# AmourWaltz/BayesLMs

Measured on AMD Instinct MI355X. Metric: train_tokens_per_sec, higher is better.
Workload: dtype f32

## Files before the change

### bayeslms_amd/csrc/blm_device.h

```cpp
#pragma once
#include <hip/hip_runtime.h>
#include <stdint.h>

#include "../../include/bayeslm.h"

#define BLM_WAVE 64

namespace blm {

struct u32x4 {
  uint32_t x, y, z, w;
};

__device__ __forceinline__ u32x4 philox4x32_10(uint32_t c0, uint32_t c1, uint32_t c2, uint32_t c3, uint32_t k0,
                                               uint32_t k1) {
  constexpr uint32_t M0 = 0xD2511F53u, M1 = 0xCD9E8D57u, W0 = 0x9E3779B9u, W1 = 0xBB67AE85u;
#pragma unroll
  for (int r = 0; r < 10; ++r) {
    const uint64_t p0 = (uint64_t)M0 * c0, p1 = (uint64_t)M1 * c2;
    const uint32_t hi0 = (uint32_t)(p0 >> 32), lo0 = (uint32_t)p0;
    const uint32_t hi1 = (uint32_t)(p1 >> 32), lo1 = (uint32_t)p1;
    const uint32_t n0 = hi1 ^ c1 ^ k0, n2 = hi0 ^ c3 ^ k1;
    c0 = n0; c1 = lo1; c2 = n2; c3 = lo0;
    k0 += W0; k1 += W1;
  }
  return {c0, c1, c2, c3};
}

__device__ __noinline__ u32x4 philox4x32_10_rolled(uint32_t c0, uint32_t c1, uint32_t c2, uint32_t c3, uint32_t k0,
                                                   uint32_t k1) {
  constexpr uint32_t M0 = 0xD2511F53u, M1 = 0xCD9E8D57u, W0 = 0x9E3779B9u, W1 = 0xBB67AE85u;
#pragma unroll 1
  for (int r = 0; r < 10; ++r) {
    const uint64_t p0 = (uint64_t)M0 * c0, p1 = (uint64_t)M1 * c2;
    const uint32_t hi0 = (uint32_t)(p0 >> 32), lo0 = (uint32_t)p0;
    const uint32_t hi1 = (uint32_t)(p1 >> 32), lo1 = (uint32_t)p1;
    const uint32_t n0 = hi1 ^ c1 ^ k0, n2 = hi0 ^ c3 ^ k1;
    c0 = n0; c1 = lo1; c2 = n2; c3 = lo0;
    k0 += W0; k1 += W1;
  }
  return {c0, c1, c2, c3};
}

__device__ __forceinline__ u32x4 philox_block(const blm_rng& r, uint64_t block) {
  return philox4x32_10((uint32_t)block, (uint32_t)(block >> 32), r.stream, r.step, (uint32_t)r.seed,
                       (uint32_t)(r.seed >> 32));
}

__device__ __forceinline__ void box_muller(uint32_t ra, uint32_t rb, float& z0, float& z1) {
  const float u1 = ((float)(ra >> 9) + 1.0f) * 1.1920928955078125e-07f;
  const float u2 = (float)(rb >> 8) * 5.9604644775390625e-08f;
  const float r = __builtin_sqrtf(-1.3862943611198906f * __builtin_amdgcn_logf(u1));
  z0 = r * __builtin_amdgcn_cosf(u2);
  z1 = r * __builtin_amdgcn_sinf(u2);
}

__device__ __forceinline__ float4 philox_normal4(const blm_rng& r, uint64_t block) {
  const u32x4 u = philox_block(r, block);
  float4 z;
  box_muller(u.x, u.y, z.x, z.y);
  box_muller(u.z, u.w, z.z, z.w);
  return z;
}

__device__ __forceinline__ float philox_normal1_rolled(const blm_rng& r, uint64_t idx) {
  const uint64_t block = idx >> 2;
  const u32x4 u = philox4x32_10_rolled((uint32_t)block, (uint32_t)(block >> 32), r.stream, r.step, (uint32_t)r.seed,
                                       (uint32_t)(r.seed >> 32));
  const bool hi = idx & 2;
  float z0, z1;
  box_muller(hi ? u.z : u.x, hi ? u.w : u.y, z0, z1);
  return (idx & 1) ? z1 : z0;
}
__device__ __forceinline__ uint32_t philox_bits1_rolled(const blm_rng& r, uint64_t idx) {
  const uint64_t block = idx >> 2;
  const u32x4 u = philox4x32_10_rolled((uint32_t)block, (uint32_t)(block >> 32), r.stream, r.step, (uint32_t)r.seed,
                                       (uint32_t)(r.seed >> 32));
  const int c = (int)(idx & 3);
  return c == 0 ? u.x : (c == 1 ? u.y : (c == 2 ? u.z : u.w));
}

__device__ __forceinline__ uint32_t dropout_threshold(float p) {
  const double t = (double)p * 4294967296.0;
  return t >= 4294967295.0 ? 0xFFFFFFFFu : (uint32_t)t;
}

__device__ __forceinline__ float wave_sum(float v) {
#pragma unroll
  for (int o = 32; o > 0; o >>= 1) v += __shfl_xor(v, o, 64);
  return v;
}
__device__ __forceinline__ float wave_max(float v) {
#pragma unroll
  for (int o = 32; o > 0; o >>= 1) v = fmaxf(v, __shfl_xor(v, o, 64));
  return v;
}

template <int NW>
__device__ __forceinline__ float block_sum(float v, float* red) {
  v = wave_sum(v);
  const int lane = threadIdx.x & 63, w = threadIdx.x >> 6;
  __syncthreads();
  if (lane == 0) red[w] = v;
  __syncthreads();
  float t = 0.f;
#pragma unroll
  for (int i = 0; i < NW; ++i) t += red[i];
  return t;
}
template <int NW>
__device__ __forceinline__ float block_max(float v, float* red) {
  v = wave_max(v);
  const int lane = threadIdx.x & 63, w = threadIdx.x >> 6;
  __syncthreads();
  if (lane == 0) red[w] = v;
  __syncthreads();
  float t = red[0];
#pragma unroll
  for (int i = 1; i < NW; ++i) t = fmaxf(t, red[i]);
  return t;
}

typedef float blm_f2 __attribute__((ext_vector_type(2)));
__device__ __forceinline__ void gelu_parts2(blm_f2 z, blm_f2& cdf, blm_f2& pdf_exp) {
  const blm_f2 x = __builtin_elementwise_abs(z) * 0.70710678118654752f;
  const blm_f2 den = __builtin_elementwise_fma(x, (blm_f2)(0.3275911f), (blm_f2)(1.0f));
  const blm_f2 t = {__builtin_amdgcn_rcpf(den.x), __builtin_amdgcn_rcpf(den.y)};
  const blm_f2 xx = -x * x;
  pdf_exp = (blm_f2){__expf(xx.x), __expf(xx.y)};
  blm_f2 poly = __builtin_elementwise_fma(t, (blm_f2)(1.061405429f), (blm_f2)(-1.453152027f));
  poly = __builtin_elementwise_fma(t, poly, (blm_f2)(1.421413741f));
  poly = __builtin_elementwise_fma(t, poly, (blm_f2)(-0.284496736f));
  poly = __builtin_elementwise_fma(t, poly, (blm_f2)(0.254829592f));
  const blm_f2 tail = (poly * t) * (0.5f * pdf_exp);
  cdf = (blm_f2){z.x >= 0.f ? 1.0f - tail.x : tail.x, z.y >= 0.f ? 1.0f - tail.y : tail.y};
}
__device__ __forceinline__ void gelu_parts(float z, float& cdf, float& pdf_exp) {
  const float x = fabsf(z) * 0.70710678118654752f;
  const float t = __builtin_amdgcn_rcpf(1.0f + 0.3275911f * x);
  pdf_exp = __expf(-x * x);
  const float poly = t * (0.254829592f + t * (-0.284496736f + t * (1.421413741f + t * (-1.453152027f + t * 1.061405429f))));
  const float tail = 0.5f * poly * pdf_exp;
  cdf = z >= 0.f ? 1.0f - tail : tail;
}
__device__ __forceinline__ float gelu_erf(float z) {
  float cdf, e;
  gelu_parts(z, cdf, e);
  return z * cdf;
}
__device__ __forceinline__ float dgelu_erf(float z) {
  float cdf, e;
  gelu_parts(z, cdf, e);
  return cdf + z * 0.3989422804014327f * e;
}

__device__ __forceinline__ float sigmoidf_(float x) { return 1.0f / (1.0f + __expf(-x)); }

__device__ __forceinline__ float gp_mix(float z, const float* coef, int N, int n) {
  return tanhf(z) * coef[n] + sigmoidf_(z) * coef[N + n] + fmaxf(z, 0.f) * coef[2 * N + n] +
         gelu_erf(z) * coef[3 * N + n];
}
__device__ __forceinline__ float dgp_mix(float z, const float* coef, int N, int n) {
  const float th = tanhf(z), sg = sigmoidf_(z);
  return (1.f - th * th) * coef[n] + sg * (1.f - sg) * coef[N + n] + (z > 0.f ? coef[2 * N + n] : 0.f) +
         dgelu_erf(z) * coef[3 * N + n];
}

}
```

### bayeslms_amd/csrc/gemm_f32_mfma.h

```cpp
#pragma once
#include <cstdlib>

#include "blm_device.h"
#include <type_traits>
#include "blm_host.h"

namespace blm {

using f32x16 = __attribute__((ext_vector_type(16))) float;

struct GemmP {
  int M, N, K;
  const float* A; long lda;
  const float* B; long ldb;
  float* C; long ldc;
  float alpha;
  unsigned flags;
  int epi;
  const float* bias;
  float* aux;
  const float* coef;
  blm_variational vb; int vb_cols;
  float* C2;
  const float* wg_mu;
// ... 183 lines not shown
  static constexpr int NREAD = ST64 ? 2 : 4;
  float v[4];
  f32x2 w[2];
  __device__ __forceinline__ void read(uint32_t base, int t) {
    if constexpr (ST64) {
#pragma unroll
      for (int h = 0; h < 2; ++h)
        asm volatile("ds_read2st64_b32 %0, %1 offset0:%2 offset1:%3" : "=v"(w[h]) : "v"(base), "n"((8 * t + 2 * h) * (S / 64)),
                     "n"((8 * t + 2 * h + 1) * (S / 64)));
    } else {
#pragma unroll
      for (int s = 0; s < 4; ++s) asm volatile("ds_read_b32 %0, %1 offset:%2" : "=v"(v[s]) : "v"(base), "n"((8 * t + s) * S * 4));
    }
  }
  __device__ __forceinline__ float get(int, int s) const {
    if constexpr (ST64) return (s & 1) ? w[s >> 1].y : w[s >> 1].x;
    else return v[s];
  }
  __device__ __forceinline__ void tie() {
    if constexpr (ST64) {
      asm volatile("" : "+v"(w[0]), "+v"(w[1]));
    } else {
#pragma unroll
      for (int s = 0; s < 4; ++s) asm volatile("" : "+v"(v[s]));
    }
  }
  __device__ __forceinline__ void add_k(f32x2 (&sum)[1]) {
    static_assert(ST64, "summed from the unpadded LDS-DMA images only");
    asm volatile("v_pk_add_f32 %0, %0, %1\n\tv_pk_add_f32 %0, %0, %2" : "+v"(sum[0]) : "v"(w[0]), "v"(w[1]));
  }
};
#ifndef BLM_GEMM_DMA
#define BLM_GEMM_DMA 1
#endif
template <int OP, int WTM, int WTN, bool SAMP, bool FAST>
constexpr bool use_dma() { return BLM_GEMM_DMA && !SAMP && FAST; }

template <int R>
__device__ __forceinline__ void r2s_kmaj_swz(float* tile, const float4 (&r)[R / 32]) {
  const int t = threadIdx.x, kq = t & 7, rr = t >> 3;
#pragma unroll
  for (int j = 0; j < R / 32; ++j) {
    const int row = rr + 32 * j;
    *reinterpret_cast<float4*>(tile + row * 32 + 4 * (kq ^ ((row >> 1) & 7))) = r[j];
  }
}

__device__ __forceinline__ void glds16(const float* gsrc, uint32_t lds_dst) {
  uint32_t keep;
  asm volatile("s_mov_b32 %0, m0\n\ts_mov_b32 m0, %2\n\ts_nop 0\n\tglobal_load_lds_dwordx4 %1, off\n\ts_mov_b32 m0, %0"
               : "=&s"(keep) : "v"(gsrc), "s"(lds_dst) : "memory");
}
__device__ __forceinline__ void glds16s(const float* sbase, uint32_t voff, uint32_t lds_dst) {
  uint32_t keep;
  asm volatile("s_mov_b32 %0, m0\n\ts_mov_b32 m0, %3\n\ts_nop 0\n\tglobal_load_lds_dwordx4 %1, %2\n\ts_mov_b32 m0, %0"
               : "=&s"(keep) : "v"(voff), "s"(sbase), "s"(lds_dst) : "memory");
}

template <int W> struct FragD {
  static constexpr int NREAD = W;
  f32x4 v[W];
  __device__ __forceinline__ void read(const uint32_t (&bt)[4], int t) {
#pragma unroll
    for (int i = 0; i < W; ++i) asm volatile("ds_read_b128 %0, %1 offset:%2" : "=v"(v[i]) : "v"(bt[t]), "n"(4096 * i));
  }
  __device__ __forceinline__ float get(int i, int s) const { return v[i][s]; }
  __device__ __forceinline__ void tie() {
#pragma unroll
    for (int i = 0; i < W; ++i) asm volatile("" : "+v"(v[i]));
  }
};

template <int N>
__device__ __forceinline__ void wait_lgkm() { asm volatile("s_waitcnt lgkmcnt(%0)" ::"n"(N > 15 ? 15 : N)); }

typedef __attribute__((ext_vector_type(2))) __bf16 bf16x2;
typedef __attribute__((ext_vector_type(8))) __bf16 bf16x8;
typedef __attribute__((ext_vector_type(4))) unsigned u32x4v;
__device__ __forceinline__ void split_bf16x8(const float (&x)[8], bf16x8& hi, bf16x8& lo) {
  u32x4v h, l;
#pragma unroll
  for (int q = 0; q < 4; ++q) {
    const f32x2 v = {x[2 * q], x[2 * q + 1]};
    const uint32_t hu = __builtin_bit_cast(uint32_t, __builtin_convertvector(v, bf16x2));
    const f32x2 r = {v.x - __uint_as_float(hu << 16), v.y - __uint_as_float(hu & 0xFFFF0000u)};
    h[q] = hu;
    l[q] = __builtin_bit_cast(uint32_t, __builtin_convertvector(r, bf16x2));
  }
  hi = __builtin_bit_cast(bf16x8, h);
  lo = __builtin_bit_cast(bf16x8, l);
}
__device__ __forceinline__ void split_bf16x8_3(const float (&x)[8], bf16x8& hi, bf16x8& mid, bf16x8& lo) {
  u32x4v h, m, l;
#pragma unroll
  for (int q = 0; q < 4; ++q) {
    const f32x2 v = {x[2 * q], x[2 * q + 1]};
    const bf16x2 hb = __builtin_convertvector(v, bf16x2);
    const f32x2 r = {v.x - (float)hb[0], v.y - (float)hb[1]};
    const bf16x2 mb = __builtin_convertvector(r, bf16x2);
    const f32x2 r2 = {r.x - (float)mb[0], r.y - (float)mb[1]};
    h[q] = __builtin_bit_cast(uint32_t, hb);
    m[q] = __builtin_bit_cast(uint32_t, mb);
    l[q] = __builtin_bit_cast(uint32_t, __builtin_convertvector(r2, bf16x2));
  }
  hi = __builtin_bit_cast(bf16x8, h);
  mid = __builtin_bit_cast(bf16x8, m);
  lo = __builtin_bit_cast(bf16x8, l);
}

__device__ __forceinline__ void gemm_keep_quad(const GemmP& p, int base_row, int row_stride, int col, float (&keep)[4]) {
  const int k = threadIdx.x & 3;
  const int m = base_row + k * row_stride;
  const int row = m / p.drop_B, b = m - row * p.drop_B;
  const uint64_t g = ((uint64_t)row * p.drop_global_cols + (uint64_t)(p.drop_col_offset + b)) * (uint64_t)p.N +
                     (uint64_t)(col & ~3);
  const u32x4 u = philox4x32_10_rolled((uint32_t)(g >> 2), (uint32_t)(g >> 34), p.drop_rng.stream, p.drop_rng.step,
                                       (uint32_t)p.drop_rng.seed, (uint32_t)(p.drop_rng.seed >> 32));
#define BLM_QUAD_BCAST(x, j) (uint32_t) __builtin_amdgcn_mov_dpp((int)(x), (j) * 0x55, 0xF, 0xF, true)
#define BLM_KEEP_FROM(j)                                                                                      \
  {                                                                                                           \
    const uint32_t w0 = BLM_QUAD_BCAST(u.x, j), w1 = BLM_QUAD_BCAST(u.y, j), w2 = BLM_QUAD_BCAST(u.z, j),     \
                   w3 = BLM_QUAD_BCAST(u.w, j);                                                               \
    const uint32_t w = k == 0 ? w0 : (k == 1 ? w1 : (k == 2 ? w2 : w3));                                      \
    keep[j] = w >= p.drop_thr ? p.drop_inv_keep : 0.f;                                                        \
  }
  BLM_KEEP_FROM(0) BLM_KEEP_FROM(1) BLM_KEEP_FROM(2) BLM_KEEP_FROM(3)
#undef BLM_KEEP_FROM
#undef BLM_QUAD_BCAST
}

__device__ __forceinline__ void gemm_keep_pair(const GemmP& p, int m, int c0, float& k0, float& k1) {
  const int row = m / p.drop_B, b = m - row * p.drop_B;
  const uint64_t g = ((uint64_t)row * p.drop_global_cols + (uint64_t)(p.drop_col_offset + b)) * (uint64_t)p.N + (uint64_t)c0;
  const u32x4 u = philox4x32_10_rolled((uint32_t)(g >> 2), (uint32_t)(g >> 34), p.drop_rng.stream, p.drop_rng.step,
                                       (uint32_t)p.drop_rng.seed, (uint32_t)(p.drop_rng.seed >> 32));
  const bool hi = g & 2;
  k0 = (hi ? u.z : u.x) >= p.drop_thr ? p.drop_inv_keep : 0.f;
  k1 = (hi ? u.w : u.y) >= p.drop_thr ? p.drop_inv_keep : 0.f;
}

__device__ __forceinline__ void gemm_eps_quad(const GemmP& p, int base_row, int row_stride, int col, float (&eps)[4]) {
  const int k = threadIdx.x & 3;
  const int rel = min(max(base_row + k * row_stride - p.vc.row_lo, 0), p.vc.srows - 1);
  const uint64_t si = (uint64_t)rel * (uint64_t)p.N + (uint64_t)(min(col, p.N - 1) & ~3);
  const u32x4 u = philox4x32_10_rolled((uint32_t)(si >> 2), (uint32_t)(si >> 34), p.vc.rng.stream, p.vc.rng.step,
                                       (uint32_t)p.vc.rng.seed, (uint32_t)(p.vc.rng.seed >> 32));
  float z0, z1, z2, z3;
  box_muller(u.x, u.y, z0, z1);
  box_muller(u.z, u.w, z2, z3);
#define BLM_QUAD_BCASTF(x, j) __int_as_float(__builtin_amdgcn_mov_dpp(__float_as_int(x), (j) * 0x55, 0xF, 0xF, true))
#define BLM_EPS_FROM(j)                                                                                   \
  {                                                                                                       \
    const float w0 = BLM_QUAD_BCASTF(z0, j), w1 = BLM_QUAD_BCASTF(z1, j), w2 = BLM_QUAD_BCASTF(z2, j),     \
                w3 = BLM_QUAD_BCASTF(z3, j);                                                              \
    eps[j] = k == 0 ? w0 : (k == 1 ? w1 : (k == 2 ? w2 : w3));                                            \
  }
  BLM_EPS_FROM(0) BLM_EPS_FROM(1) BLM_EPS_FROM(2) BLM_EPS_FROM(3)
#undef BLM_EPS_FROM
#undef BLM_QUAD_BCASTF
}

template <int EPI>
__device__ __forceinline__ void epi_elem(const GemmP& p, bool accum, int row, int col, float acc, float bias, float keep, bool kl_on = true, bool atomic = false) {
  const long o = (long)row * p.ldc + col;
  float v = p.alpha * acc;
  if constexpr (EPI == BLM_EPI_BIAS) {
    if (kl_on) v += bias;
  } else if constexpr (EPI == BLM_EPI_BIAS_GELU) {
    v += bias;
    float cdf, e;
    gelu_parts(v, cdf, e);
    if (p.aux) p.aux[o] = (cdf + v * 0.3989422804014327f * e) * keep;
    v = v * cdf * keep;
  } else if constexpr (EPI == BLM_EPI_MUL_DGELU) {
    v *= p.aux[o];
  } else if constexpr (EPI == BLM_EPI_GP_MIX) {
    v += bias;
    if (p.aux) p.aux[o] = v;
    v = gp_mix(v, p.coef, p.N, col) * keep;
  } else if constexpr (EPI == BLM_EPI_MUL_DGP_MIX) {
    v *= keep;
    if (p.C2) p.C2[o] = v;
    v *= dgp_mix(p.aux[o], p.coef, p.N, col);
  } else if constexpr (EPI == BLM_EPI_BAYES_WGRAD) {
    const float dW = v;
    const int rel = row - p.vc.row_lo;
    if ((unsigned)rel < (unsigned)p.vc.srows) {
      const long si = (long)rel * p.N + col;
      const float sig = __expf(p.vc.lgstd[si]);
      float e;
      if (p.vc.eps) e = p.vc.eps[si];
      else if (p.eps_quad) e = keep;
      else e = philox_normal1_rolled(p.vc.rng, (uint64_t)si);
      const float klw = kl_on ? p.kl_lambda * p.kl_inv_n : 0.f;
      const float g2 = dW * e * sig + klw * (sig * sig - 1.0f);
      if (atomic) atomicAdd(p.C2 + si, g2);
      else p.C2[si] = accum ? p.C2[si] + g2 : g2;
      v = dW + klw * p.wg_mu[o];
    }
  }
  if constexpr (EPI == BLM_EPI_NONE || EPI == BLM_EPI_BIAS || EPI == BLM_EPI_BAYES_WGRAD) {
    if (atomic) { atomicAdd(p.C + o, v); return; }
  }
  p.C[o] = accum ? p.C[o] + v : v;
}

template <int EPI, int WTM, int WTN>
__device__ __forceinline__ void epilogue(const GemmP& p, f32x16 (&acc)[WTM][WTN], int m0, int n0, int wm, int wn,
                                         int li, int lh, bool kl_on = true, bool atomic = false) {
  constexpr bool DROP = (EPI == BLM_EPI_BIAS_GELU || EPI == BLM_EPI_GP_MIX || EPI == BLM_EPI_MUL_DGP_MIX);
  constexpr bool BIAS = (EPI == BLM_EPI_BIAS || EPI == BLM_EPI_BIAS_GELU || EPI == BLM_EPI_GP_MIX);
  const bool accum = p.flags & BLM_GEMM_ACCUMULATE;
  int col[WTN];
  float bias[WTN];
#pragma unroll
  for (int j = 0; j < WTN; ++j) {
    col[j] = n0 + wn * (32 * WTN) + ((INTERLEAVE && WTN == 2) ? 2 * li + j : 32 * j + li);
    bias[j] = 0.f;
    if constexpr (BIAS) bias[j] = col[j] < p.N ? p.bias[col[j]] : 0.f;
  }
  const bool pair_store = INTERLEAVE && WTN == 2 && (EPI == BLM_EPI_NONE || EPI == BLM_EPI_BIAS) && !atomic && (p.ldc % 2 == 0) &&
                          ((reinterpret_cast<uintptr_t>(p.C) & 7) == 0);
#pragma unroll
  for (int i = 0; i < WTM; ++i) {
#pragma unroll
    for (int rq = 0; rq < 4; ++rq) {
      const int mrow0 = 8 * rq + 4 * lh;
      const int row0 = m0 + wm * (32 * WTM) + ((INTERLEAVE && WTM == 2) ? 2 * mrow0 + i : 32 * i + mrow0);
      constexpr int RS = (INTERLEAVE && WTM == 2) ? 2 : 1;
      float keep[4][WTN];
#pragma unroll
      for (int rr = 0; rr < 4; ++rr)
#pragma unroll
        for (int j = 0; j < WTN; ++j) keep[rr][j] = 1.f;
      if constexpr (EPI == BLM_EPI_BAYES_WGRAD) {
        if (p.eps_quad) {
#pragma unroll
          for (int j = 0; j < WTN; ++j) {
            float e4[4];
            gemm_eps_quad(p, row0, RS, col[j], e4);
#pragma unroll
            for (int rr = 0; rr < 4; ++rr) keep[rr][j] = e4[rr];
          }
        }
      }
      if constexpr (DROP) {
        if (p.drop_on) {
          if (INTERLEAVE && WTN == 2 && p.drop_quad) {
#pragma unroll
            for (int rr = 0; rr < 4; ++rr) gemm_keep_pair(p, row0 + rr * RS, min(col[0], p.N - 2), keep[rr][0], keep[rr][WTN - 1]);
          } else if (!(INTERLEAVE && WTN == 2) && p.drop_quad) {
#pragma unroll
            for (int j = 0; j < WTN; ++j) {
              float k4[4];
              gemm_keep_quad(p, row0, RS, col[j], k4);
#pragma unroll
              for (int rr = 0; rr < 4; ++rr) keep[rr][j] = k4[rr];
            }
          } else {
#pragma unroll
            for (int rr = 0; rr < 4; ++rr)
#pragma unroll
              for (int j = 0; j < WTN; ++j) keep[rr][j] = gemm_keep(p, row0 + rr * RS, min(col[j], p.N - 1));
          }
        }
      }
#pragma unroll
      for (int rr = 0; rr < 4; ++rr) {
        const int row = row0 + rr * RS;
        const int r = 4 * rq + rr;
        if (row >= p.M) continue;
        if constexpr (WTN == 2) {
          if (pair_store && col[1] < p.N) {
            float2* dst = reinterpret_cast<float2*>(p.C + (long)row * p.ldc + col[0]);
            float2 v = make_float2(p.alpha * acc[i][0][r] + bias[0], p.alpha * acc[i][1][r] + bias[1]);
            if (accum) { const float2 old = *dst; v.x += old.x; v.y += old.y; }
            *dst = v;
            continue;
          }
        }
#pragma unroll
        for (int j = 0; j < WTN; ++j)
          if (col[j] < p.N) epi_elem<EPI>(p, accum, row, col[j], acc[i][j][r], bias[j], keep[rr][j], kl_on, atomic);
      }
    }
  }
  BLM_PROF_WG_END();
}

__device__ __forceinline__ void store4(float* dst, const float4& v) { *reinterpret_cast<float4*>(dst) = v; }

template <int EPI, int WTM, int WTN, int WGN = 2>
__device__ __forceinline__ void epilogue_rows(const GemmP& p, f32x16 (&acc)[WTM][WTN], float* stage, int m0, int n0,
                                              int wm, int wn, int li, int lh) {
  constexpr int BN = 32 * WTN * WGN, SS = BN + 4;
  constexpr int NP = WTM == 2 ? 2 : 1;
  constexpr int TPRW = BN / 4, RPS = (128 * WGN) / TPRW;
  const int t = threadIdx.x, c4 = 4 * (t % TPRW);
  const int col = n0 + c4;
  const bool accum = p.flags & BLM_GEMM_ACCUMULATE;
  float4 bias = make_float4(0.f, 0.f, 0.f, 0.f);
  if constexpr (EPI == BLM_EPI_BIAS || EPI == BLM_EPI_BIAS_GELU || EPI == BLM_EPI_GP_MIX || EPI == BLM_EPI_CE_PART || EPI == BLM_EPI_MC_PART)
    if (col < p.N && p.bias) bias = *reinterpret_cast<const float4*>(p.bias + col);
#pragma unroll
  for (int pass = 0; pass < NP; ++pass) {
    __syncthreads();
    if (WTM == 1 || wm == pass) {
#pragma unroll
      for (int i = 0; i < WTM; ++i)
#pragma unroll
        for (int j = 0; j < WTN; ++j)
#pragma unroll
          for (int r = 0; r < 16; ++r) {
            const int lrow = (WTM == 2 ? 32 * i : 32 * wm) + (r & 3) + 8 * (r >> 2) + 4 * lh;
            stage[lrow * SS + wn * (32 * WTN) + 32 * j + li] = p.alpha * acc[i][j][r];
          }
    }
    __syncthreads();
    if constexpr (EPI == BLM_EPI_CE_PART) {
      const bool valid = col < p.ce_nv;
      const bool part = valid && col + 4 > p.ce_nv;
      for (int lr = t / TPRW; lr < 64; lr += RPS) {
        const int row = m0 + 64 * pass + lr;
        if (row >= p.M) break;
        float4 v = *reinterpret_cast<const float4*>(stage + lr * SS + c4);
        v.x += bias.x; v.y += bias.y; v.z += bias.z; v.w += bias.w;
        if (part) {
          if (col + 1 >= p.ce_nv) v.y = -INFINITY;
          if (col + 2 >= p.ce_nv) v.z = -INFINITY;
          v.w = -INFINITY;
        }
        float m = valid ? fmaxf(fmaxf(v.x, v.y), fmaxf(v.z, v.w)) : -INFINITY;
#pragma unroll
        for (int o = TPRW / 2; o > 0; o >>= 1) m = fmaxf(m, __shfl_xor(m, o, 64));
        float sum = valid ? (__expf(v.x - m) + __expf(v.y - m)) + (__expf(v.z - m) + __expf(v.w - m)) : 0.f;
#pragma unroll
        for (int o = TPRW / 2; o > 0; o >>= 1) sum += __shfl_xor(sum, o, 64);
        if (t % TPRW == 0) {
          float* d = p.aux + ((long)row * p.gn + n0 / BN) * 2;
          d[0] = m;
          d[1] = sum;
        }
        const long long tg = p.ce_tgt[row >> p.ce_row_shift];
        if (valid && tg >= col && tg < col + 4 && tg < p.ce_nv) p.ce_tlogit[row] = tg == col ? v.x : (tg == col + 1 ? v.y : (tg == col + 2 ? v.z : v.w));
      }
    } else if constexpr (EPI == BLM_EPI_MC_PART) {
      const int sh = p.ce_row_shift, S = p.mc_s;
      const bool keep = p.epi == BLM_EPI_MC_LOGP;
      const float logS = __logf((float)S);
      const bool valid = col < p.ce_nv;
      const bool in1 = col + 1 < p.ce_nv, in2 = col + 2 < p.ce_nv, in3 = col + 3 < p.ce_nv;
      for (int g = t / TPRW; g < (64 >> sh); g += RPS) {
        const int row0 = m0 + 64 * pass + (g << sh);
        if (row0 >= p.M) break;
        float hs = 0.f, ms = 0.f;
        if (valid) {
          const float* z = stage + (g << sh) * SS + c4;
          const float* lse = p.mc_lse + row0;
          float4 r = make_float4(-INFINITY, -INFINITY, -INFINITY, -INFINITY);
          for (int s = 0; s < S; ++s) {
            const float4 v = *reinterpret_cast<const float4*>(z + s * SS);
            const float l = lse[s];
            r.x = fmaxf(r.x, v.x + bias.x - l); r.y = fmaxf(r.y, v.y + bias.y - l);
            r.z = fmaxf(r.z, v.z + bias.z - l); r.w = fmaxf(r.w, v.w + bias.w - l);
          }
          float4 sw = make_float4(0.f, 0.f, 0.f, 0.f), su = sw;
          for (int s = 0; s < S; ++s) {
            const float4 v = *reinterpret_cast<const float4*>(z + s * SS);
            const float l = lse[s];
            const float ux = v.x + bias.x - l - r.x, uy = v.y + bias.y - l - r.y, uz = v.z + bias.z - l - r.z, uw = v.w + bias.w - l - r.w;
            const float wx = __expf(ux), wy = __expf(uy), wz = __expf(uz), ww = __expf(uw);
            sw.x += wx; sw.y += wy; sw.z += wz; sw.w += ww;
            su.x = fmaf(wx, ux, su.x); su.y = fmaf(wy, uy, su.y); su.z = fmaf(wz, uz, su.z); su.w = fmaf(ww, uw, su.w);
          }
          const float invS = 1.f / S;
          auto col_terms = [&](float rr, float W, float U, bool in) {
            const float L = __logf(W) - logS, er = __expf(rr);
            if (in) {
              hs = fmaf(er * W * invS, rr + L, hs);
              ms = fmaf(er, fmaf(-L, W, U), ms);
            }
            return rr + L;
          };
          float4 lp;
          lp.x = col_terms(r.x, sw.x, su.x, true);
          lp.y = col_terms(r.y, sw.y, su.y, in1);
          lp.z = col_terms(r.z, sw.z, su.z, in2);
          lp.w = col_terms(r.w, sw.w, su.w, in3);
          if (keep) {
            float* d = p.C + (long)(row0 >> sh) * p.ldc + col;
            if (in3) {
              store4(d, lp);
            } else {
              d[0] = lp.x;
              if (in1) d[1] = lp.y;
              if (in2) d[2] = lp.z;
            }
          }
        }
#pragma unroll
        for (int o = TPRW / 2; o > 0; o >>= 1) {
          hs += __shfl_xor(hs, o, 64);
          ms += __shfl_xor(ms, o, 64);
        }
        if (t % TPRW == 0) {
          float* d = p.aux + ((long)(row0 >> sh) * p.gn + n0 / BN) * 2;
          d[0] = hs;
          d[1] = ms;
        }
      }
    } else if (col < p.N) {
      auto keep4 = [&](int row) {
        float4 kp = make_float4(1.f, 1.f, 1.f, 1.f);
        if (p.drop_on) {
          const int rr = row / p.drop_B, b = row - rr * p.drop_B;
          const uint64_t g = ((uint64_t)rr * p.drop_global_cols + (uint64_t)(p.drop_col_offset + b)) * (uint64_t)p.N + (uint64_t)col;
          const u32x4 u = philox4x32_10((uint32_t)(g >> 2), (uint32_t)(g >> 34), p.drop_rng.stream, p.drop_rng.step,
                                        (uint32_t)p.drop_rng.seed, (uint32_t)(p.drop_rng.seed >> 32));
          kp = make_float4(u.x >= p.drop_thr ? p.drop_inv_keep : 0.f, u.y >= p.drop_thr ? p.drop_inv_keep : 0.f,
                           u.z >= p.drop_thr ? p.drop_inv_keep : 0.f, u.w >= p.drop_thr ? p.drop_inv_keep : 0.f);
        }
        return kp;
      };
      auto row_body = [&](int lr, const float4& a) {
        const int row = m0 + 64 * pass + lr;
        float4 v = *reinterpret_cast<const float4*>(stage + lr * SS + c4);
        const long o = (long)row * p.ldc + col;
        if constexpr (EPI == BLM_EPI_BIAS) {
          v.x += bias.x; v.y += bias.y; v.z += bias.z; v.w += bias.w;
        } else if constexpr (EPI == BLM_EPI_GP_MIX) {
          const float4 kp = keep4(row);
          v.x += bias.x; v.y += bias.y; v.z += bias.z; v.w += bias.w;
          if (p.aux) store4(p.aux + o, v);
          v.x = gp_mix(v.x, p.coef, p.N, col) * kp.x;
          v.y = gp_mix(v.y, p.coef, p.N, col + 1) * kp.y;
          v.z = gp_mix(v.z, p.coef, p.N, col + 2) * kp.z;
          v.w = gp_mix(v.w, p.coef, p.N, col + 3) * kp.w;
        } else if constexpr (EPI == BLM_EPI_MUL_DGP_MIX) {
          const float4 kp = keep4(row);
          v.x *= kp.x; v.y *= kp.y; v.z *= kp.z; v.w *= kp.w;
          if (p.C2) store4(p.C2 + o, v);
          v.x *= dgp_mix(a.x, p.coef, p.N, col);
          v.y *= dgp_mix(a.y, p.coef, p.N, col + 1);
          v.z *= dgp_mix(a.z, p.coef, p.N, col + 2);
          v.w *= dgp_mix(a.w, p.coef, p.N, col + 3);
        } else if constexpr (EPI == BLM_EPI_BIAS_GELU) {
          const float4 kp = keep4(row);
          float4 d;
          {
            const blm_f2 z0 = (blm_f2){v.x, v.y} + (blm_f2){bias.x, bias.y}, z1 = (blm_f2){v.z, v.w} + (blm_f2){bias.z, bias.w};
            const blm_f2 k0 = {kp.x, kp.y}, k1 = {kp.z, kp.w};
            blm_f2 c0, e0, c1, e1;
            gelu_parts2(z0, c0, e0);
            gelu_parts2(z1, c1, e1);
            const blm_f2 d0 = __builtin_elementwise_fma(z0 * 0.3989422804014327f, e0, c0) * k0, y0 = (z0 * c0) * k0;
            const blm_f2 d1 = __builtin_elementwise_fma(z1 * 0.3989422804014327f, e1, c1) * k1, y1 = (z1 * c1) * k1;
            d = make_float4(d0.x, d0.y, d1.x, d1.y);
            v = make_float4(y0.x, y0.y, y1.x, y1.y);
          }
          if (p.aux) store4(p.aux + o, d);
        } else if constexpr (EPI == BLM_EPI_MUL_DGELU) {
          v.x *= a.x; v.y *= a.y; v.z *= a.z; v.w *= a.w;
        }
        float4* dst = reinterpret_cast<float4*>(p.C + o);
        if (accum) { const float4 old = *dst; v.x += old.x; v.y += old.y; v.z += old.z; v.w += old.w; }
#ifdef BLM_GEMM_LIFE
        if (blm_dbg_store == 1) { if (v.x == 1.2345e-30f) store4(p.C + o, v); return; }
        if (blm_dbg_store == 2) { store4(p.C + (long)(lr + 64 * pass) * p.ldc + c4, v); return; }
#endif
        store4(p.C + o, v);
      };
      if constexpr (EPI == BLM_EPI_MUL_DGELU || EPI == BLM_EPI_MUL_DGP_MIX) {
        constexpr int NIT = 64 / RPS;
        float4 ax[NIT];
#pragma unroll
        for (int i = 0; i < NIT; ++i) {
          const int row = m0 + 64 * pass + t / TPRW + RPS * i;
          ax[i] = row < p.M ? *reinterpret_cast<const float4*>(p.aux + (long)row * p.ldc + col) : make_float4(0.f, 0.f, 0.f, 0.f);
        }
#pragma unroll
        for (int i = 0; i < NIT; ++i) {
          const int lr = t / TPRW + RPS * i;
          if (m0 + 64 * pass + lr < p.M) row_body(lr, ax[i]);
        }
      } else {
        const float4 none = make_float4(0.f, 0.f, 0.f, 0.f);
        for (int lr = t / TPRW; lr < 64; lr += RPS) {
          if (m0 + 64 * pass + lr >= p.M) break;
          row_body(lr, none);
        }
      }
    }
  }
  BLM_PROF_WG_END();
}

template <int OP, int WTM, int WTN, bool SAMP, bool FAST, int SPLIT = 0, int WGN = 2>
__global__ __launch_bounds__(128 * WGN, WGN == 2 ? 2 : 1) void gemm_f32_kernel(const GemmP p) {
  constexpr int BM = 64 * WTM, BN = 32 * WTN * WGN, NT = 128 * WGN;
  constexpr bool A_KMAJ = (OP != BLM_GEMM_TN), B_KMAJ = (OP == BLM_GEMM_NT);
  constexpr bool DMA = use_dma<OP, WTM, WTN, SAMP, FAST>();
  constexpr int SA = BM + (DMA ? 0 : 4), SB = BN + (DMA ? 0 : 4);
  constexpr int KSX = DMA ? 32 : KS;
  constexpr int TA = A_KMAJ ? BM * KSX : BK * SA, TB = B_KMAJ ? BN * KSX : BK * SB;
  constexpr int NA = BM / 32, NB = BN / 32;
  extern __shared__ __attribute__((aligned(16))) float smem[];
  float* const As = smem;
  float* const Bs = smem + 2 * TA;

  const int nb = p.gm * p.gn;
  const bool whole = (int)blockIdx.x < p.tail_from;
  const int ntail = nb - p.tail_from, rtail = (int)blockIdx.x - p.tail_from;
  const int bid = whole ? (int)blockIdx.x : p.tail_from + rtail % ntail, ks = whole ? 0 : rtail / ntail;
  const bool atomic = p.atomic && !whole;
  const int q = nb >> 3, rem = nb & 7, xcd = bid & 7;
  const int id = (xcd < rem ? xcd * (q + 1) : rem * (q + 1) + (xcd - rem) * q) + (bid >> 3);
  constexpr int GROUP = 8;
  int mt, nt;
  if (p.gn <= GROUP) {
    mt = id / p.gn;
    nt = id - mt * p.gn;
  } else {
    const int per = GROUP * p.gn, grp = id / per, first = grp * GROUP, gsz = min(p.gm - first, GROUP), in = id - grp * per;
    mt = first + in % gsz;
    nt = in / gsz;
  }
  const int m0 = mt * BM, n0 = nt * BN;

  const int t = threadIdx.x, lane = t & 63, wave = t >> 6;
  const int wm = wave / WGN, wn = wave % WGN, li = lane & 31, lh = lane >> 5;
#ifdef BLM_GEMM_LIFE
  if (t == 0 && blockIdx.x < 8192) {
    blm_wg_life[4 * blockIdx.x] = wall_clock64();
    blm_wg_life[4 * blockIdx.x + 2] = (long long)__builtin_amdgcn_s_getreg((31 << 11) | 4) |
                                      ((long long)__builtin_amdgcn_s_getreg((31 << 11) | 20) << 32);
  }
#endif

  float4 ra[NA], rb[NB], rl[SAMP ? NB : 1];
  const float* pa[FAST ? NA : 1];
  const float* pb[FAST ? NB : 1];
  const float* pl[(FAST && SAMP) ? NB : 1];
  bool in_slice[(FAST && SAMP) ? NB : 1];
  long stepA = 0, stepB = 0, stepL = 0;

  if constexpr (FAST) {
    if constexpr (A_KMAJ) {
#pragma unroll
      for (int j = 0; j < NA; ++j) pa[j] = p.A + (long)min(m0 + (t >> 3) + 32 * j, p.M - 1) * p.lda + 4 * (t & 7);
      stepA = BK;
    } else {
      constexpr int TPR = BM / 4, RPP = 256 / TPR;
#pragma unroll
      for (int j = 0; j < NA; ++j) pa[j] = p.A + (long)(t / TPR + RPP * j) * p.lda + min(m0 + 4 * (t % TPR), p.M - 4);
      stepA = (long)BK * p.lda;
    }
    if constexpr (B_KMAJ) {
#pragma unroll
      for (int j = 0; j < NB; ++j) {
        const int n = min(n0 + (t >> 3) + 32 * j, p.N - 1);
        pb[j] = p.B + (long)n * p.ldb + 4 * (t & 7);
        if constexpr (SAMP) {
          const int rel = n - p.vb.row_lo;
          in_slice[j] = (unsigned)rel < (unsigned)p.vb.srows;
          pl[j] = p.vb.lgstd + (long)min(max(rel, 0), p.vb.srows - 1) * p.vb_cols + 4 * (t & 7);
        }
      }
      stepB = BK;
      stepL = BK;
    } else {
      constexpr int TPR = BN / 4, RPP = 256 / TPR;
#pragma unroll
      for (int j = 0; j < NB; ++j) {
        const int c = min(n0 + 4 * (t % TPR), p.N - 4);
        pb[j] = p.B + (long)(t / TPR + RPP * j) * p.ldb + c;
        if constexpr (SAMP) pl[j] = p.vb.lgstd + c;
      }
      stepB = (long)BK * p.ldb;
    }
  }

  float4 cs = make_float4(0.f, 0.f, 0.f, 0.f);
  const bool do_cs = !A_KMAJ && p.colsum_a != nullptr && n0 == 0;

  auto fetch_fast = [&](int kt) {
    if constexpr (FAST) {
#pragma unroll
      for (int j = 0; j < NA; ++j) ra[j] = *reinterpret_cast<const float4*>(pa[j] + kt * stepA);
#pragma unroll
      for (int j = 0; j < NB; ++j) rb[j] = *reinterpret_cast<const float4*>(pb[j] + kt * stepB);
      if constexpr (SAMP) {
        if constexpr (B_KMAJ) {
#pragma unroll
          for (int j = 0; j < NB; ++j) rl[j] = *reinterpret_cast<const float4*>(pl[j] + kt * stepL);
        } else {
          constexpr int TPR = BN / 4, RPP = 256 / TPR;
#pragma unroll
          for (int j = 0; j < NB; ++j) {
            const int rel = kt * BK + t / TPR + RPP * j - p.vb.row_lo;
            in_slice[j] = (unsigned)rel < (unsigned)p.vb.srows;
            rl[j] = *reinterpret_cast<const float4*>(pl[j] + (long)min(max(rel, 0), p.vb.srows - 1) * p.vb_cols);
          }
        }
      }
    }
  };
  auto fetch_slow = [&](int k0) {
    const bool av = p.a_vec, bv = p.b_vec;
    if constexpr (A_KMAJ) g2r_kmaj<BM>(p.A, p.lda, m0, p.M, k0, p.K, av, ra);
    else g2r_nmaj<BM>(p.A, p.lda, k0, p.K, m0, p.M, av, ra);
    if constexpr (B_KMAJ) g2r_kmaj<BN>(p.B, p.ldb, n0, p.N, k0, p.K, bv, rb);
    else g2r_nmaj<BN>(p.B, p.ldb, k0, p.K, n0, p.N, bv, rb);
    if constexpr (SAMP) {
      if constexpr (B_KMAJ) g2r_kmaj<BN>(p.vb.lgstd, p.vb_cols, n0 - p.vb.row_lo, p.vb.srows, k0, p.K, true, rl);
      else g2r_nmaj<BN>(p.vb.lgstd, p.vb_cols, k0 - p.vb.row_lo, p.vb.srows, n0, p.N, true, rl);
    }
  };
  auto stash = [&](int buf, int k0, bool fast) {
    float* At = As + buf * TA;
    float* Bt = Bs + buf * TB;
    if constexpr (SAMP) {
#pragma unroll
      for (int j = 0; j < NB; ++j) {
        int srow, scol;
        if constexpr (B_KMAJ) { srow = n0 + (t >> 3) + 32 * j; scol = k0 + 4 * (t & 7); }
        else { constexpr int TPR = BN / 4, RPP = 256 / TPR; srow = k0 + t / TPR + RPP * j; scol = n0 + 4 * (t % TPR); }
        if constexpr (FAST) {
          if (fast) {
            if constexpr (B_KMAJ) srow = min(srow, p.N - 1); else scol = min(scol, p.N - 4);
            if (in_slice[j]) rb[j] = sample4(rb[j], rl[j], p.vb, p.vb_cols, srow, scol);
            continue;
          }
        }
        rb[j] = sample4(rb[j], rl[j], p.vb, p.vb_cols, srow, scol);
      }
    }
    if constexpr (!A_KMAJ && !DMA) {
      if (do_cs) {
#pragma unroll
        for (int j = 0; j < NA; ++j) { cs.x += ra[j].x; cs.y += ra[j].y; cs.z += ra[j].z; cs.w += ra[j].w; }
      }
    }
    if constexpr (DMA) {
      if constexpr (A_KMAJ) r2s_kmaj_swz<BM>(At, ra); else r2s_nmaj<BM, SA>(At, ra);
      if constexpr (B_KMAJ) r2s_kmaj_swz<BN>(Bt, rb); else r2s_nmaj<BN, SB>(Bt, rb);
    } else {
      if constexpr (A_KMAJ) r2s_kmaj<BM>(At, ra); else r2s_nmaj<BM, SA>(At, ra);
      if constexpr (B_KMAJ) r2s_kmaj<BN>(Bt, rb); else r2s_nmaj<BN, SB>(Bt, rb);
    }
  };

  f32x16 acc[WTM][WTN];
#pragma unroll
  for (int i = 0; i < WTM; ++i)
#pragma unroll
    for (int j = 0; j < WTN; ++j) acc[i][j] = (f32x16)(0.f);

  auto compute = [&](int cur, auto&& mid) {
    using FA = FragG<A_KMAJ, WTM, SA>;
    using FB = FragG<B_KMAJ, WTN, SB>;
    const uint32_t a_base = A_KMAJ ? lds_u32(As + cur * TA + (wm * (32 * WTM) + li) * KS + 4 * lh)
                                   : lds_u32(As + cur * TA + (4 * lh) * SA + wm * (32 * WTM) + li);
    const uint32_t b_base = B_KMAJ ? lds_u32(Bs + cur * TB + (wn * (32 * WTN) + li) * KS + 4 * lh)
                                   : lds_u32(Bs + cur * TB + (4 * lh) * SB + wn * (32 * WTN) + li);
    FA a[2];
    FB b[2];
    a[0].read(a_base, 0);
    b[0].read(b_base, 0);
#pragma unroll
    for (int t4 = 0; t4 < 4; ++t4) {
      if (t4 + 1 < 4) {
        a[(t4 + 1) & 1].read(a_base, t4 + 1);
        b[(t4 + 1) & 1].read(b_base, t4 + 1);
        wait_lgkm<FA::NREAD + FB::NREAD>();
      } else {
        wait_lgkm<0>();
      }
      a[t4 & 1].tie();
      b[t4 & 1].tie();
      if (t4 == 2) mid();
      __builtin_amdgcn_sched_barrier(0);
#pragma unroll
      for (int s4 = 0; s4 < 4; ++s4)
#pragma unroll
        for (int i = 0; i < WTM; ++i)
#pragma unroll
          for (int j = 0; j < WTN; ++j)
            acc[i][j] = __builtin_amdgcn_mfma_f32_32x32x2f32(a[t4 & 1].get(i, s4), b[t4 & 1].get(j, s4), acc[i][j], 0, 0, 0);
    }
  };

  const int swz = (li >> 1) & 7;
  constexpr bool CS_FRAG = DMA && !A_KMAJ && SPLIT == 0, CS_WALK = DMA && !A_KMAJ && SPLIT != 0;
  struct CsOff {};
  struct CsPartials { f32x2 p[WTM]; int wn; };
  typename std::conditional<CS_FRAG, CsPartials, CsOff>::type csf;
  if constexpr (CS_FRAG) {
#pragma unroll
    for (int i = 0; i < WTM; ++i) csf.p[i] = (f32x2)(0.f);
    csf.wn = do_cs ? __builtin_amdgcn_readfirstlane(wn) : -1;
  }
  typename std::conditional<CS_WALK, float, CsOff>::type cs1{};
  auto compute_dma = [&](int cur) {
    if constexpr (DMA) {
      if constexpr (CS_WALK) {
        if (do_cs && t < BM) {
          const float* col = As + cur * TA + t;
#pragma unroll 8
          for (int k = 0; k < BK; ++k) cs1 += col[k * SA];
        }
      }
      using FA = typename std::conditional<A_KMAJ, FragD<WTM>, FragG<false, WTM, SA>>::type;
      using FB = typename std::conditional<B_KMAJ, FragD<WTN>, FragG<false, WTN, SB>>::type;
      uint32_t abt[4], bbt[4];
      const uint32_t a0 = A_KMAJ ? lds_u32(As + cur * TA + (wm * (32 * WTM) + li) * 32) : lds_u32(As + cur * TA + (4 * lh) * SA + wm * (32 * WTM) + li);
      const uint32_t b0 = B_KMAJ ? lds_u32(Bs + cur * TB + (wn * (32 * WTN) + li) * 32) : lds_u32(Bs + cur * TB + (4 * lh) * SB + wn * (32 * WTN) + li);
#pragma unroll
      for (int t4 = 0; t4 < 4; ++t4) {
        const uint32_t ch = (uint32_t)(((2 * t4 + lh) ^ swz) * 16);
        abt[t4] = a0 + ch;
        bbt[t4] = b0 + ch;
      }
      auto rd_a = [&](FA& f, int t4) { if constexpr (A_KMAJ) f.read(abt, t4); else f.read(a0, t4); };
      auto rd_b = [&](FB& f, int t4) { if constexpr (B_KMAJ) f.read(bbt, t4); else f.read(b0, t4); };
      if constexpr (SPLIT != 0) {
        FA a[4];
        FB b[4];
        rd_a(a[0], 0); rd_b(b[0], 0); rd_a(a[1], 1); rd_b(b[1], 1);
        rd_a(a[2], 2); rd_b(b[2], 2); rd_a(a[3], 3); rd_b(b[3], 3);
#pragma unroll
        for (int g = 0; g < 2; ++g) {
          constexpr int PEND = 2 * (FA::NREAD + FB::NREAD);
          if (g == 0) wait_lgkm<(PEND > 15 ? 15 : PEND)>(); else wait_lgkm<0>();
          a[2 * g].tie(); a[2 * g + 1].tie(); b[2 * g].tie(); b[2 * g + 1].tie();
          float xa[WTM][8], xb[WTN][8];
#pragma unroll
          for (int i = 0; i < WTM; ++i)
#pragma unroll
            for (int s4 = 0; s4 < 4; ++s4) { xa[i][s4] = a[2 * g].get(i, s4); xa[i][4 + s4] = a[2 * g + 1].get(i, s4); }
#pragma unroll
          for (int j = 0; j < WTN; ++j)
#pragma unroll
            for (int s4 = 0; s4 < 4; ++s4) { xb[j][s4] = b[2 * g].get(j, s4); xb[j][4 + s4] = b[2 * g + 1].get(j, s4); }
          if constexpr (SPLIT == 6) {
            bf16x8 ah[WTM], am[WTM], al[WTM], bh[WTN], bm[WTN], bl[WTN];
#pragma unroll
            for (int i = 0; i < WTM; ++i) split_bf16x8_3(xa[i], ah[i], am[i], al[i]);
#pragma unroll
            for (int j = 0; j < WTN; ++j) split_bf16x8_3(xb[j], bh[j], bm[j], bl[j]);
#pragma unroll
            for (int i = 0; i < WTM; ++i)
#pragma unroll
              for (int j = 0; j < WTN; ++j) {
                acc[i][j] = __builtin_amdgcn_mfma_f32_32x32x16_bf16(al[i], bh[j], acc[i][j], 0, 0, 0);
                acc[i][j] = __builtin_amdgcn_mfma_f32_32x32x16_bf16(ah[i], bl[j], acc[i][j], 0, 0, 0);
                acc[i][j] = __builtin_amdgcn_mfma_f32_32x32x16_bf16(am[i], bm[j], acc[i][j], 0, 0, 0);
                acc[i][j] = __builtin_amdgcn_mfma_f32_32x32x16_bf16(am[i], bh[j], acc[i][j], 0, 0, 0);
                acc[i][j] = __builtin_amdgcn_mfma_f32_32x32x16_bf16(ah[i], bm[j], acc[i][j], 0, 0, 0);
                acc[i][j] = __builtin_amdgcn_mfma_f32_32x32x16_bf16(ah[i], bh[j], acc[i][j], 0, 0, 0);
              }
          } else {
            bf16x8 ah[WTM], al[WTM], bh[WTN], bl[WTN];
#pragma unroll
            for (int i = 0; i < WTM; ++i) split_bf16x8(xa[i], ah[i], al[i]);
#pragma unroll
            for (int j = 0; j < WTN; ++j) split_bf16x8(xb[j], bh[j], bl[j]);
#pragma unroll
            for (int i = 0; i < WTM; ++i)
#pragma unroll
              for (int j = 0; j < WTN; ++j) {
                acc[i][j] = __builtin_amdgcn_mfma_f32_32x32x16_bf16(al[i], bh[j], acc[i][j], 0, 0, 0);
                acc[i][j] = __builtin_amdgcn_mfma_f32_32x32x16_bf16(ah[i], bl[j], acc[i][j], 0, 0, 0);
                acc[i][j] = __builtin_amdgcn_mfma_f32_32x32x16_bf16(ah[i], bh[j], acc[i][j], 0, 0, 0);
              }
          }
        }
        return;
      }
      FA a[2];
      FB b[2];
      rd_a(a[0], 0);
      rd_b(b[0], 0);
#pragma unroll
      for (int t4 = 0; t4 < 4; ++t4) {
        if (t4 + 1 < 4) {
          rd_a(a[(t4 + 1) & 1], t4 + 1);
          rd_b(b[(t4 + 1) & 1], t4 + 1);
          wait_lgkm<FA::NREAD + FB::NREAD>();
        } else {
          wait_lgkm<0>();
        }
        a[t4 & 1].tie();
        b[t4 & 1].tie();
        if constexpr (CS_FRAG) {
          int sel = csf.wn;
// ... 338 lines not shown
```

Measured before the change: 414,400.

## Prefetch epilogue aux/accum loads, incrementalize dropout offsets, use bitop3 xor in Philox

```diff
diff --git a/bayeslms_amd/csrc/blm_device.h b/bayeslms_amd/csrc/blm_device.h
--- a/bayeslms_amd/csrc/blm_device.h
+++ b/bayeslms_amd/csrc/blm_device.h
@@ -12,6 +12,13 @@
   uint32_t x, y, z, w;
 };
 
+__device__ __forceinline__ uint32_t xor3_skey(uint32_t a, uint32_t b, uint32_t k) {
+  uint32_t r;
+  asm("v_bitop3_b32 %0, %1, %2, %3 bitop3:0x96" : "=v"(r) : "v"(a), "v"(b), "s"(k));
+  return r;
+}
+
+template <bool SKEY = false>
 __device__ __forceinline__ u32x4 philox4x32_10(uint32_t c0, uint32_t c1, uint32_t c2, uint32_t c3, uint32_t k0,
                                                uint32_t k1) {
   constexpr uint32_t M0 = 0xD2511F53u, M1 = 0xCD9E8D57u, W0 = 0x9E3779B9u, W1 = 0xBB67AE85u;
@@ -20,7 +27,9 @@
     const uint64_t p0 = (uint64_t)M0 * c0, p1 = (uint64_t)M1 * c2;
     const uint32_t hi0 = (uint32_t)(p0 >> 32), lo0 = (uint32_t)p0;
     const uint32_t hi1 = (uint32_t)(p1 >> 32), lo1 = (uint32_t)p1;
-    const uint32_t n0 = hi1 ^ c1 ^ k0, n2 = hi0 ^ c3 ^ k1;
+    uint32_t n0, n2;
+    if (SKEY && r >= 2) n0 = xor3_skey(hi1, c1, k0); else n0 = hi1 ^ c1 ^ k0;
+    if (SKEY && r >= 1) n2 = xor3_skey(hi0, c3, k1); else n2 = hi0 ^ c3 ^ k1;
     c0 = n0; c1 = lo1; c2 = n2; c3 = lo0;
     k0 += W0; k1 += W1;
   }
diff --git a/bayeslms_amd/csrc/gemm_f32_mfma.h b/bayeslms_amd/csrc/gemm_f32_mfma.h
--- a/bayeslms_amd/csrc/gemm_f32_mfma.h
+++ b/bayeslms_amd/csrc/gemm_f32_mfma.h
@@ -509,6 +509,41 @@
   float4 bias = make_float4(0.f, 0.f, 0.f, 0.f);
   if constexpr (EPI == BLM_EPI_BIAS || EPI == BLM_EPI_BIAS_GELU || EPI == BLM_EPI_GP_MIX || EPI == BLM_EPI_CE_PART || EPI == BLM_EPI_MC_PART)
     if (col < p.N && p.bias) bias = *reinterpret_cast<const float4*>(p.bias + col);
+  constexpr bool ROWS = EPI != BLM_EPI_CE_PART && EPI != BLM_EPI_MC_PART;
+  constexpr bool AUX = EPI == BLM_EPI_MUL_DGELU || EPI == BLM_EPI_MUL_DGP_MIX;
+  constexpr bool DROP = EPI == BLM_EPI_BIAS_GELU || EPI == BLM_EPI_GP_MIX || EPI == BLM_EPI_MUL_DGP_MIX;
+  constexpr int NIT = 64 / RPS;
+  const int lr0 = t / TPRW;
+  constexpr bool OLDB = ROWS && !DROP;
+  const bool batch = ROWS && (AUX || (OLDB && accum));
+  float4 ax[NIT], old[NIT];
+#pragma unroll
+  for (int i = 0; i < NIT; ++i) ax[i] = old[i] = make_float4(0.f, 0.f, 0.f, 0.f);
+  auto request = [&](int pass) {
+    if constexpr (ROWS) {
+      if (batch && col < p.N) {
+#pragma unroll
+        for (int i = 0; i < NIT; ++i) {
+          const int row = m0 + 64 * pass + lr0 + RPS * i;
+          const long o = (long)row * p.ldc + col;
+          if constexpr (AUX) ax[i] = row < p.M ? *reinterpret_cast<const float4*>(p.aux + o) : make_float4(0.f, 0.f, 0.f, 0.f);
+          if constexpr (OLDB) old[i] = (accum && row < p.M) ? *reinterpret_cast<const float4*>(p.C + o) : make_float4(0.f, 0.f, 0.f, 0.f);
+        }
+      }
+    }
+  };
+  constexpr bool EARLY = WTM == 2;
+  if constexpr (EARLY) request(0);
+  uint64_t dg = 0, dstep = 0, dwrap = 0;
+  int db = 0, drs = 0;
+  if constexpr (DROP) {
+    if (p.drop_on) {
+      const int qs = RPS / p.drop_B;
+      drs = RPS - qs * p.drop_B;
+      dstep = ((uint64_t)qs * (uint64_t)p.drop_global_cols + (uint64_t)drs) * (uint64_t)p.N;
+      dwrap = ((uint64_t)p.drop_global_cols - (uint64_t)p.drop_B) * (uint64_t)p.N;
+    }
+  }
 #pragma unroll
   for (int pass = 0; pass < NP; ++pass) {
     __syncthreads();
@@ -523,6 +558,7 @@
             stage[lrow * SS + wn * (32 * WTN) + 32 * j + li] = p.alpha * acc[i][j][r];
           }
     }
+    if constexpr (!EARLY) request(0);
     __syncthreads();
     if constexpr (EPI == BLM_EPI_CE_PART) {
       const bool valid = col < p.ce_nv;
@@ -617,26 +653,35 @@
         }
       }
     } else if (col < p.N) {
-      auto keep4 = [&](int row) {
+      if constexpr (DROP) {
+        if (p.drop_on) {
+          const int row = m0 + 64 * pass + lr0, rr = row / p.drop_B;
+          db = row - rr * p.drop_B;
+          dg = ((uint64_t)rr * p.drop_global_cols + (uint64_t)(p.drop_col_offset + db)) * (uint64_t)p.N + (uint64_t)col;
+        }
+      }
+      auto keep4 = [&]() {
         float4 kp = make_float4(1.f, 1.f, 1.f, 1.f);
         if (p.drop_on) {
-          const int rr = row / p.drop_B, b = row - rr * p.drop_B;
-          const uint64_t g = ((uint64_t)rr * p.drop_global_cols + (uint64_t)(p.drop_col_offset + b)) * (uint64_t)p.N + (uint64_t)col;
-          const u32x4 u = philox4x32_10((uint32_t)(g >> 2), (uint32_t)(g >> 34), p.drop_rng.stream, p.drop_rng.step,
-                                        (uint32_t)p.drop_rng.seed, (uint32_t)(p.drop_rng.seed >> 32));
+          const uint64_t g = dg;
+          db += drs;
+          dg += dstep;
+          if (db >= p.drop_B) { db -= p.drop_B; dg += dwrap; }
+          const u32x4 u = philox4x32_10<true>((uint32_t)(g >> 2), (uint32_t)(g >> 34), p.drop_rng.stream, p.drop_rng.step,
+                                              (uint32_t)p.drop_rng.seed, (uint32_t)(p.drop_rng.seed >> 32));
           kp = make_float4(u.x >= p.drop_thr ? p.drop_inv_keep : 0.f, u.y >= p.drop_thr ? p.drop_inv_keep : 0.f,
                            u.z >= p.drop_thr ? p.drop_inv_keep : 0.f, u.w >= p.drop_thr ? p.drop_inv_keep : 0.f);
         }
         return kp;
       };
-      auto row_body = [&](int lr, const float4& a) {
+      auto row_body = [&](int lr, const float4 a, const float4 old) {
         const int row = m0 + 64 * pass + lr;
         float4 v = *reinterpret_cast<const float4*>(stage + lr * SS + c4);
         const long o = (long)row * p.ldc + col;
         if constexpr (EPI == BLM_EPI_BIAS) {
           v.x += bias.x; v.y += bias.y; v.z += bias.z; v.w += bias.w;
         } else if constexpr (EPI == BLM_EPI_GP_MIX) {
-          const float4 kp = keep4(row);
+          const float4 kp = keep4();
           v.x += bias.x; v.y += bias.y; v.z += bias.z; v.w += bias.w;
           if (p.aux) store4(p.aux + o, v);
           v.x = gp_mix(v.x, p.coef, p.N, col) * kp.x;
@@ -644,7 +689,7 @@
           v.z = gp_mix(v.z, p.coef, p.N, col + 2) * kp.z;
           v.w = gp_mix(v.w, p.coef, p.N, col + 3) * kp.w;
         } else if constexpr (EPI == BLM_EPI_MUL_DGP_MIX) {
-          const float4 kp = keep4(row);
+          const float4 kp = keep4();
           v.x *= kp.x; v.y *= kp.y; v.z *= kp.z; v.w *= kp.w;
           if (p.C2) store4(p.C2 + o, v);
           v.x *= dgp_mix(a.x, p.coef, p.N, col);
@@ -652,7 +697,7 @@
           v.z *= dgp_mix(a.z, p.coef, p.N, col + 2);
           v.w *= dgp_mix(a.w, p.coef, p.N, col + 3);
         } else if constexpr (EPI == BLM_EPI_BIAS_GELU) {
-          const float4 kp = keep4(row);
+          const float4 kp = keep4();
           float4 d;
           {
             const blm_f2 z0 = (blm_f2){v.x, v.y} + (blm_f2){bias.x, bias.y}, z1 = (blm_f2){v.z, v.w} + (blm_f2){bias.z, bias.w};
@@ -670,34 +715,32 @@
           v.x *= a.x; v.y *= a.y; v.z *= a.z; v.w *= a.w;
         }
         float4* dst = reinterpret_cast<float4*>(p.C + o);
-        if (accum) { const float4 old = *dst; v.x += old.x; v.y += old.y; v.z += old.z; v.w += old.w; }
+        if constexpr (OLDB) {
+          if (accum) { v.x += old.x; v.y += old.y; v.z += old.z; v.w += old.w; }
+        } else {
+          if (accum) { const float4 c = *dst; v.x += c.x; v.y += c.y; v.z += c.z; v.w += c.w; }
+        }
 #ifdef BLM_GEMM_LIFE
         if (blm_dbg_store == 1) { if (v.x == 1.2345e-30f) store4(p.C + o, v); return; }
         if (blm_dbg_store == 2) { store4(p.C + (long)(lr + 64 * pass) * p.ldc + c4, v); return; }
 #endif
         store4(p.C + o, v);
       };
-      if constexpr (EPI == BLM_EPI_MUL_DGELU || EPI == BLM_EPI_MUL_DGP_MIX) {
-        constexpr int NIT = 64 / RPS;
-        float4 ax[NIT];
+      if (batch) {
 #pragma unroll
         for (int i = 0; i < NIT; ++i) {
-          const int row = m0 + 64 * pass + t / TPRW + RPS * i;
-          ax[i] = row < p.M ? *reinterpret_cast<const float4*>(p.aux + (long)row * p.ldc + col) : make_float4(0.f, 0.f, 0.f, 0.f);
-        }
-#pragma unroll
-        for (int i = 0; i < NIT; ++i) {
-          const int lr = t / TPRW + RPS * i;
-          if (m0 + 64 * pass + lr < p.M) row_body(lr, ax[i]);
+          const int lr = lr0 + RPS * i;
+          if (m0 + 64 * pass + lr < p.M) row_body(lr, ax[i], old[i]);
         }
       } else {
         const float4 none = make_float4(0.f, 0.f, 0.f, 0.f);
-        for (int lr = t / TPRW; lr < 64; lr += RPS) {
+        for (int lr = lr0; lr < 64; lr += RPS) {
           if (m0 + 64 * pass + lr >= p.M) break;
-          row_body(lr, none);
-        }
-      }
-    }
+          row_body(lr, none, none);
+        }
+      }
+    }
+    if (pass + 1 < NP) request(pass + 1);
   }
   BLM_PROF_WG_END();
 }
```

Measured after the change: 414,300. Within noise of the previous version (-0.0%).
